# alibaba/unified-audio

Hardware: AMD Instinct MI355X
Metric: audio-seconds/sec H-Codec encode+decode @16kHz b=32 (higher is better)
Workload: dtype f32

## Files before the change

unified_audio_amd/csrc/conv_gemm.hip:

```cpp
#include <algorithm>
#include <cstdlib>
#include <type_traits>

#include "common.h"
#include "split_planes.h"

#ifndef QA_LOAD_AT
#define QA_LOAD_AT 0
#endif

#ifdef QA_TIMING
__device__ unsigned long long g_qa_timing[10];
extern "C" int qa_debug_timing(unsigned long long* out, int reset) {
    if (out && hipMemcpyFromSymbol(out, HIP_SYMBOL(g_qa_timing), sizeof(g_qa_timing)) != hipSuccess) return -1;
    if (reset) {
        unsigned long long z[10] = {0};
        if (hipMemcpyToSymbol(HIP_SYMBOL(g_qa_timing), z, sizeof(z)) != hipSuccess) return -1;
    }
    return 0;
}
#endif

namespace qa {

// ... 12 lines not shown
        f(std::integral_constant<int, I>{});
        static_for<N, I + 1>(f);
    }
}

constexpr int TAP_WIN = 8;

__device__ __forceinline__ float snake_f(float x, float a) {
    const float s = sinf(a * x);
    return x + s * s / (a + 1e-9f);
}
__device__ __forceinline__ f32x4 snake4(f32x4 v, const float* alpha, int n) {
    const f32x4 a = *reinterpret_cast<const f32x4*>(alpha + n);
    const f32x4 r = {snake_f(v.x, a.x), snake_f(v.y, a.y), snake_f(v.z, a.z), snake_f(v.w, a.w)};
    return r;
}

__device__ __forceinline__ f32x4 epilogue4(f32x4 v, const ConvParams& p, long long m, int n, f32x4 bias, f32x4 gamma) {
    v += bias;
    if (p.gate) {
        const f32x4 g = *reinterpret_cast<const f32x4*>(p.gate + m * p.ldg + n);
        v.x *= silu_f(g.x); v.y *= silu_f(g.y); v.z *= silu_f(g.z); v.w *= silu_f(g.w);
    }
    if (p.act == ACT_SNAKE) {
        v = snake4(v, p.alpha, n);
    } else if (p.act != ACT_NONE) {
        v.x = apply_act(v.x, p.act); v.y = apply_act(v.y, p.act); v.z = apply_act(v.z, p.act); v.w = apply_act(v.w, p.act);
    }
    if (p.gamma) v *= gamma;
    if (p.res) v += *reinterpret_cast<const f32x4*>(p.res + m * p.ldr + n);
    if (p.post_act == ACT_SNAKE) {
        v = snake4(v, p.alpha, n);
    } else if (p.post_act != ACT_NONE) {
        v.x = apply_act(v.x, p.post_act); v.y = apply_act(v.y, p.post_act); v.z = apply_act(v.z, p.post_act);
        v.w = apply_act(v.w, p.post_act);
    }
    if (p.y2) *reinterpret_cast<f32x4*>(p.y2 + m * p.ldy2 + n) = snake4(v, p.alpha2, n);
    if (p.rope && n < p.rope_n) {
        const int t = p.rope_pos0 + (int)(m % p.rope_T), i = (n % p.rope_hd) >> 1;
        const f32x4 cs = *reinterpret_cast<const f32x4*>(p.rope + ((long long)t * (p.rope_hd >> 1) + i) * 2);
        const f32x4 r = {v.x * cs.x - v.y * cs.y, v.y * cs.x + v.x * cs.y, v.z * cs.z - v.w * cs.w, v.w * cs.z + v.z * cs.w};
        v = r;
    }
    return v;
}

template <int BM, int BN, int WM, int WN, bool PRO_ELU, int BK = 32, bool LINEAR = false, int NPL = 0, bool PRE = false>
__global__ __launch_bounds__(256, conv_gemm_min_wg(BM, BN, BK, NPL > 0)) void conv_gemm_kernel(const ConvParams p_in) {
    constexpr bool SPLIT = NPL > 0;
    constexpr int NP = SPLIT ? NPL : 3;
    static_assert(NPL >= 0 && NPL <= 3, "0 = fp32 chain, else the number of bf16 planes");
    static_assert(SPLIT || !PRE, "a pre-split weight image feeds the bf16-plane instances only");
    ConvParams p = p_in;
    constexpr int LDS = BK + 4;
    constexpr int RPP = 256 / (BK / 4);
    constexpr int WTM = BM / WM, WTN = BN / WN;
    constexpr int TM = WTM / 32, TN = WTN / 32;
    constexpr int A_IT = BM / RPP, B_IT = BN / RPP;
    static_assert(WM * WN == 4, "4 waves per workgroup");
    static_assert(TM >= 1 && TN >= 1, "wave tile must hold at least one 32x32 MFMA tile");

    constexpr int SMEM_FLOATS = SPLIT ? 2 * (BM + BN) * 3 * BK / 2 : 2 * (BM + BN) * LDS;
    __shared__ __attribute__((aligned(16))) float smem[SMEM_FLOATS];
    __shared__ int s_tap[BM * TAP_WIN];
    float* sA = smem;
    float* sB = smem + 2 * BM * LDS;
    constexpr int PLANE_A = BM * BK * 2, PLANE_B = BN * BK * 2;
    constexpr int BUF_BYTES = 3 * (PLANE_A + PLANE_B);
    char* const sbytes = reinterpret_cast<char*>(smem);
    auto swz = [](int row, int slot) { return BK == 16 ? slot ^ ((row >> 3) & 1) : slot ^ ((row >> 2) & 3); };

    const int tid = threadIdx.x, lane = tid & 63, wave = tid >> 6;
    const int wm = wave / WN, wn = wave % WN;
    const int tiles_n = (p.N + BN - 1) / BN;
    int tile = blockIdx.x;
    if (p.xcd_swizzle) {
        const int nwg = gridDim.x, q = nwg >> 3, r = nwg & 7;
        const int xcd = tile & 7, local = tile >> 3;
        tile = (xcd < r ? xcd * (q + 1) : r * (q + 1) + (xcd - r) * q) + local;
    }
    int tm_i = tile / tiles_n, tn_i = tile % tiles_n;
    if (p.panel > 0 && tiles_n > p.panel) {
        const int tiles_m = (p.M + BM - 1) / BM;
        const int per_panel = tiles_m * p.panel;
        const int panel = tile / per_panel, r = tile - panel * per_panel;
        const int pw = min(p.panel, tiles_n - panel * p.panel);
        tm_i = r / pw;
        tn_i = panel * p.panel + (r - tm_i * pw);
    }
    const int m0 = tm_i * BM;
    const int n0 = tn_i * BN;

    const int ld_row = tid / (BK / 4);
    const int ld_c4 = (tid % (BK / 4)) * 4;

    const bool reflect = p.pad_mode == PAD_REFLECT;
    const int ldx_i = (int)p.ldx;
    const int t_virtual = p.T_in * (p.in_rep > 1 ? p.in_rep : 1);
    const int dil = p.dilation > 1 ? p.dilation : 1;
    auto build_taps = [&](int jbase) {
        for (int e = tid; e < BM * TAP_WIN; e += 256) {
            const int row = e / TAP_WIN, j = jbase + (e % TAP_WIN);
            const int m = min(m0 + row, p.M - 1);
            const int t = m % p.T_out;
            int len = t_virtual, lp = p.Lp;
            if (p.lens) {
                len = min(p.lens[m / p.T_out] * p.len_mul, t_virtual);
                lp = len <= p.max_pad ? p.max_pad + 1 : len;
            }
            int r = t * p.stride - p.pad_left + j * dil;
            const int rr = r < 0 ? -r : (r >= lp ? 2 * (lp - 1) - r : r);
            r = reflect ? rr : r;
            const bool ok = r >= 0 && r < len && j < p.ksize;
            const unsigned ru = ok ? (unsigned)r : 0u;
            const unsigned src = __umulhi(ru, p.rep_magic) + ru * p.rep_one;
            s_tap[e] = ok ? (int)(src * (unsigned)ldx_i) : -1;
        }
    };
    if (!LINEAR) build_taps(0);
    int jbase = 0;

    const float* a_ptr[A_IT];
    int a_tab[A_IT];
#pragma unroll
    for (int i = 0; i < A_IT; ++i) {
        const int m = min(m0 + ld_row + RPP * i, p.M - 1);
        a_ptr[i] = LINEAR ? p.x + (long long)m * p.ldx + ld_c4 : p.x + (long long)(m / p.T_out) * p.T_in * p.ldx + ld_c4;
        a_tab[i] = (ld_row + RPP * i) * TAP_WIN;
    }
    const float* b_ptr[B_IT];
    if constexpr (!PRE) {
#pragma unroll
        for (int i = 0; i < B_IT; ++i) {
            const int n = min(n0 + ld_row + RPP * i, p.N - 1);
            b_ptr[i] = p.w + (long long)n * p.K + ld_c4;
        }
    }
    constexpr int BP_BLOCK = 16 * NP;
    constexpr int BP_UNITS = BN * BK / 128 * BP_BLOCK, BP_IT = PRE ? BP_UNITS / 256 : 1;
    static_assert(!PRE || (BN == 128 && BP_UNITS % 256 == 0), "the image path exists for the 128-column tiles: every thread moves BP_IT whole units");
    const char* bp_ptr[BP_IT];
    int bp_lds[BP_IT];
    if constexpr (PRE) {
#pragma unroll
        for (int i = 0; i < BP_IT; ++i) {
            const int u = tid + 256 * i, v = u % BP_BLOCK;
            const int pl = v >> 4, slot = v % (BK / 8);
            const int row = u / BP_BLOCK * (128 / BK) + (v & 15) / (BK / 8);
            const int n = min(n0 + row, p.N - 1);
            bp_ptr[i] = static_cast<const char*>(p.wp) + plane_byte_offset((long long)n * p.K + slot * 8, pl);
            bp_lds[i] = 3 * PLANE_A + pl * PLANE_B + row * BK * 2 + swz(row, slot) * 16;
        }
    }
    const int nk = p.K / BK;

    f32x16 acc[TM][TN];
#pragma unroll
    for (int i = 0; i < TM; ++i)
#pragma unroll
        for (int j = 0; j < TN; ++j)
#pragma unroll
            for (int r = 0; r < 16; ++r) acc[i][j][r] = 0.f;

    f32x4 a_reg[A_IT], b_reg[B_IT];
    u32x4 bp_reg[BP_IT];
    float a_keep[A_IT];

#define QA_LOAD_GLOBAL(KC)                                                                                     \
    {                                                                                                          \
        const int k0_ = (KC) * BK;                                                                             \
        if (LINEAR) {                                                                                          \
            _Pragma("unroll") for (int i = 0; i < A_IT; ++i) a_reg[i] = *reinterpret_cast<const f32x4*>(a_ptr[i] + k0_); \
        } else {                                                                                               \
            const int j_ = k0_ / p.C_in;                                                                       \
            const int c_ = k0_ - j_ * p.C_in;                                                                  \
            if (j_ >= jbase + TAP_WIN) {                          \
                jbase = j_;                                                                                    \
                build_taps(jbase);                                                                             \
                __syncthreads();                                                                               \
            }                                                                                                  \
            _Pragma("unroll") for (int i = 0; i < A_IT; ++i) {                                                 \
                const int off_ = s_tap[a_tab[i] + (j_ - jbase)];                                               \
                a_keep[i] = off_ >= 0 ? 1.f : 0.f;                                                             \
                a_reg[i] = *reinterpret_cast<const f32x4*>(a_ptr[i] + (unsigned)(max(off_, 0) + c_));          \
            }                                                                                                  \
        }                                                                                                      \
        if constexpr (PRE) {                                                                                   \
            _Pragma("unroll") for (int i = 0; i < BP_IT; ++i)                                                  \
                bp_reg[i] = *reinterpret_cast<const u32x4*>(bp_ptr[i] + (long long)(KC) * (BK * 6)); \
        } else {                                                                                               \
            _Pragma("unroll") for (int i = 0; i < B_IT; ++i) b_reg[i] = *reinterpret_cast<const f32x4*>(b_ptr[i] + k0_); \
        }                                                                                                      \
    }
#define QA_STORE_LDS(BUF)                                                                                      \
    { if constexpr (SPLIT) {                                                                                   \
        char* a_ = sbytes + (BUF) * BUF_BYTES;                                                                 \
        const int sl_ = ld_c4 >> 3, in_ = (ld_c4 & 7) * 2;                                                     \
        _Pragma("unroll") for (int i = 0; i < A_IT; ++i) {                                                     \
            f32x4 v = LINEAR ? a_reg[i] : a_reg[i] * a_keep[i];                                                \
            if (PRO_ELU) {                                                                                     \
                v.x = elu_f(v.x); v.y = elu_f(v.y); v.z = elu_f(v.z); v.w = elu_f(v.w);                        \
            }                                                                                                  \
            u32x2 h_, m_, l_;                                                                                  \
            split4_planes<NP>(v, h_, m_, l_);                                                                  \
            const int r_ = ld_row + RPP * i, o_ = r_ * BK * 2 + swz(r_, sl_) * 16 + in_;                       \
            *reinterpret_cast<u32x2*>(a_ + o_) = h_;                                                           \
            if constexpr (NP >= 2) *reinterpret_cast<u32x2*>(a_ + PLANE_A + o_) = m_;                          \
            if constexpr (NP == 3) *reinterpret_cast<u32x2*>(a_ + 2 * PLANE_A + o_) = l_;                      \
        }                                                                                                      \
        if constexpr (PRE) {                                                                                   \
            _Pragma("unroll") for (int i = 0; i < BP_IT; ++i)                                                  \
                *reinterpret_cast<u32x4*>(a_ + bp_lds[i]) = bp_reg[i];                                         \
        } else {                                                                                               \
        char* b_ = a_ + 3 * PLANE_A;                                                                           \
        _Pragma("unroll") for (int i = 0; i < B_IT; ++i) {                                                     \
            u32x2 h_, m_, l_;                                                                                  \
            split4_planes<NP>(b_reg[i], h_, m_, l_);                                                           \
            const int r_ = ld_row + RPP * i, o_ = r_ * BK * 2 + swz(r_, sl_) * 16 + in_;                       \
            *reinterpret_cast<u32x2*>(b_ + o_) = h_;                                                           \
            if constexpr (NP >= 2) *reinterpret_cast<u32x2*>(b_ + PLANE_B + o_) = m_;                          \
            if constexpr (NP == 3) *reinterpret_cast<u32x2*>(b_ + 2 * PLANE_B + o_) = l_;                      \
        } }                                                                                                    \
    } else {                                                                                                   \
        float* a_ = sA + (BUF) * BM * LDS;                                                                     \
        float* b_ = sB + (BUF) * BN * LDS;                                                                     \
        _Pragma("unroll") for (int i = 0; i < A_IT; ++i) {                                                     \
            f32x4 v = LINEAR ? a_reg[i] : a_reg[i] * a_keep[i];                                                \
            if (PRO_ELU) {                                                                                     \
                v.x = elu_f(v.x); v.y = elu_f(v.y); v.z = elu_f(v.z); v.w = elu_f(v.w);                        \
            }                                                                                                  \
            *reinterpret_cast<f32x4*>(a_ + (ld_row + RPP * i) * LDS + ld_c4) = v;                              \
        }                                                                                                      \
        _Pragma("unroll") for (int i = 0; i < B_IT; ++i)                                                       \
            *reinterpret_cast<f32x4*>(b_ + (ld_row + RPP * i) * LDS + ld_c4) = b_reg[i];                       \
    } }

    __syncthreads();
    QA_LOAD_GLOBAL(0)
    QA_STORE_LDS(0)
    __syncthreads();

    const int frag_row = lane & 31;
    const int frag_k = (lane >> 5) * 4;
#ifdef QA_TIMING
    const long long tbegin = __builtin_readcyclecounter();
    const unsigned long long rbegin = __builtin_amdgcn_s_memrealtime();
#endif
    constexpr int NKK = BK / 8;
    if constexpr (SPLIT) {
        constexpr int NG = BK / 16;
        const int sl_h = lane >> 5;
        int a_off[TM], b_off[TN];
#pragma unroll
        for (int i = 0; i < TM; ++i) {
            const int r = wm * WTM + i * 32 + frag_row;
            a_off[i] = r * BK * 2 + swz(r, sl_h) * 16;
        }
#pragma unroll
        for (int j = 0; j < TN; ++j) {
            const int r = wn * WTN + j * 32 + frag_row;
            b_off[j] = 3 * PLANE_A + r * BK * 2 + swz(r, sl_h) * 16;
        }
        for (int kc = 0; kc < nk; ++kc) {
            const int cur = kc & 1;
            const int nxt = min(kc + 1, nk - 1);
            const char* base = sbytes + cur * BUF_BYTES;
#pragma unroll
            for (int g = 0; g < NG; ++g) {
                bf16x8 af[NP][TM], bf[NP][TN];
#pragma unroll
                for (int pl = 0; pl < NP; ++pl) {
#pragma unroll
                    for (int i = 0; i < TM; ++i)
                        af[pl][i] = *reinterpret_cast<const bf16x8*>(base + pl * PLANE_A + (a_off[i] ^ (32 * g)));
#pragma unroll
                    for (int j = 0; j < TN; ++j)
                        bf[pl][j] = *reinterpret_cast<const bf16x8*>(base + pl * PLANE_B + (b_off[j] ^ (32 * g)));
                }
                if (g == 0) QA_LOAD_GLOBAL(nxt)
                if (g == NG - 1) QA_STORE_LDS(cur ^ 1)
                if constexpr (NP == 3) {
#pragma unroll
                for (int q = 0; q < 6; ++q)
#pragma unroll
                    for (int i = 0; i < TM; ++i)
#pragma unroll
                        for (int j = 0; j < TN; ++j)
                            acc[i][j] = __builtin_amdgcn_mfma_f32_32x32x16_bf16(bf[PAIR_B[q]][j], af[PAIR_A[q]][i], acc[i][j], 0, 0, 0);
                } else {
                    static_for<6>([&](auto q_c) {
                        constexpr int q = decltype(q_c)::value;
                        if constexpr (pair_kept(q, NP)) {
#pragma unroll
                            for (int i = 0; i < TM; ++i)
#pragma unroll
                                for (int j = 0; j < TN; ++j)
                                    acc[i][j] = __builtin_amdgcn_mfma_f32_32x32x16_bf16(bf[PAIR_B[q]][j], af[PAIR_A[q]][i], acc[i][j], 0, 0, 0);
                        }
                    });
                }
                __builtin_amdgcn_sched_barrier(0);
            }
            __syncthreads();
        }
    } else
    for (int kc = 0; kc < nk; ++kc) {
        const int cur = kc & 1;
        const int nxt = min(kc + 1, nk - 1);
        const float* a = sA + cur * BM * LDS + (wm * WTM + frag_row) * LDS + frag_k;
        const float* b = sB + cur * BN * LDS + (wn * WTN + frag_row) * LDS + frag_k;
        f32x4 af[2][TM], bf[2][TN];
#pragma unroll
        for (int i = 0; i < TM; ++i) af[0][i] = *reinterpret_cast<const f32x4*>(a + i * 32 * LDS);
#pragma unroll
        for (int j = 0; j < TN; ++j) bf[0][j] = *reinterpret_cast<const f32x4*>(b + j * 32 * LDS);
#pragma unroll
        for (int kk = 0; kk < NKK; ++kk) {
            const int cb = kk & 1, nb = cb ^ 1;
            if (kk < NKK - 1) {
#pragma unroll
                for (int i = 0; i < TM; ++i) af[nb][i] = *reinterpret_cast<const f32x4*>(a + i * 32 * LDS + (kk + 1) * 8);
#pragma unroll
                for (int j = 0; j < TN; ++j) bf[nb][j] = *reinterpret_cast<const f32x4*>(b + j * 32 * LDS + (kk + 1) * 8);
            }
            if (kk == QA_LOAD_AT) QA_LOAD_GLOBAL(nxt)
            if (kk == NKK - 1) QA_STORE_LDS(cur ^ 1)
#pragma unroll
            for (int i = 0; i < TM; ++i)
#pragma unroll
                for (int j = 0; j < TN; ++j) {
                    acc[i][j] = __builtin_amdgcn_mfma_f32_32x32x2f32(bf[cb][j].x, af[cb][i].x, acc[i][j], 0, 0, 0);
                    acc[i][j] = __builtin_amdgcn_mfma_f32_32x32x2f32(bf[cb][j].y, af[cb][i].y, acc[i][j], 0, 0, 0);
                    acc[i][j] = __builtin_amdgcn_mfma_f32_32x32x2f32(bf[cb][j].z, af[cb][i].z, acc[i][j], 0, 0, 0);
                    acc[i][j] = __builtin_amdgcn_mfma_f32_32x32x2f32(bf[cb][j].w, af[cb][i].w, acc[i][j], 0, 0, 0);
                }
            __builtin_amdgcn_sched_barrier(0);
        }
        __syncthreads();
    }
#ifdef QA_TIMING
    const long long tloop = __builtin_readcyclecounter();
#endif
#undef QA_LOAD_GLOBAL
#undef QA_STORE_LDS

    constexpr int EP_LD = BN + 4;
    constexpr int EP_ROWS = WM * 32;
    constexpr int EP_C4 = BN / 4;
    static_assert(EP_ROWS * EP_LD <= 2 * (BM + BN) * LDS, "epilogue staging must fit in the operand buffers");
    static_assert(256 % EP_C4 == 0, "a thread keeps its column group across iterations");
    static_assert(EP_C4 % 8 == 0, "arg-min epilogue: the 8 lanes of a 32-column group are consecutive lanes of one wave");
    float* stage = smem;
    const int row_l = lane & 31, col_h = 4 * (lane >> 5);
    const int ep_c4 = tid % EP_C4, ep_r0 = tid / EP_C4;
    const int ep_n = n0 + 4 * ep_c4;
    const f32x4 zero4 = {0.f, 0.f, 0.f, 0.f}, one4 = {1.f, 1.f, 1.f, 1.f};
    f32x4 bias4 = zero4, gamma4 = one4;
    if (p.vec_epi && ep_n < p.N) {
        if (p.bias) bias4 = *reinterpret_cast<const f32x4*>(p.bias + ep_n);
        if (p.gamma) gamma4 = *reinterpret_cast<const f32x4*>(p.gamma + ep_n);
    }
    static_for<TM>([&](auto i_c) {
        constexpr int i = decltype(i_c)::value;
        __syncthreads();
#pragma unroll
        for (int j = 0; j < TN; ++j)
#pragma unroll
            for (int g = 0; g < 4; ++g) {
                const f32x4 v = {acc[i][j][4 * g], acc[i][j][4 * g + 1], acc[i][j][4 * g + 2], acc[i][j][4 * g + 3]};
                *reinterpret_cast<f32x4*>(stage + (wm * 32 + row_l) * EP_LD + wn * WTN + j * 32 + 8 * g + col_h) = v;
            }
        __syncthreads();
#pragma unroll 1
        for (int r = ep_r0; r < EP_ROWS; r += 256 / EP_C4) {
            const long long m = m0 + (r >> 5) * WTM + i * 32 + (r & 31);
            if (p.am_dist) {
                float best = INFINITY;
                int bi = 0x7fffffff;
                if (m < p.M && ep_n < p.N) {
                    const f32x4 sv = *reinterpret_cast<const f32x4*>(stage + r * EP_LD + 4 * ep_c4);
                    const f32x4 e4 = *reinterpret_cast<const f32x4*>(p.am_e2 + ep_n);
                    const float xx = p.am_x2[m];
#pragma unroll
                    for (int e = 0; e < 4; ++e) {
                        const float dist = (xx - 2.f * sv[e]) + e4[e];
                        if (dist < best) {
                            best = dist;
                            bi = ep_n + e;
                        }
                    }
                }
#pragma unroll
                for (int o = 1; o < 8; o <<= 1) {
                    const float d2 = __shfl_xor(best, o, 64);
                    const int i2 = __shfl_xor(bi, o, 64);
                    if (d2 < best || (d2 == best && i2 < bi)) {
                        best = d2;
                        bi = i2;
                    }
                }
                if ((ep_c4 & 7) == 0 && m < p.M && ep_n < p.N) {
                    p.am_dist[m * p.am_ld + (ep_n >> 5)] = best;
                    p.am_idx[m * p.am_ld + (ep_n >> 5)] = bi;
                }
                continue;
            }
            if (m >= p.M || ep_n >= p.N) continue;
            f32x4 v = *reinterpret_cast<const f32x4*>(stage + r * EP_LD + 4 * ep_c4);
            if (p.vec_epi) {
                v = epilogue4(v, p, m, ep_n, bias4, gamma4);
                *reinterpret_cast<f32x4*>(p.y + m * p.ldy + ep_n) = v;
            } else {
                for (int e = 0; e < 4 && ep_n + e < p.N; ++e) {
                    const int n = ep_n + e;
                    float u = v[e] + (p.bias ? p.bias[n] : 0.f);
                    if (p.gate) u = silu_f(p.gate[m * p.ldg + n]) * u;
                    u = apply_act(u, p.act);
                    if (p.gamma) u *= p.gamma[n];
                    if (p.res) u += p.res[m * p.ldr + n];
                    u = apply_act(u, p.post_act);
                    p.y[m * p.ldy + n] = u;
                }
            }
        }
// ... 1 lines not shown
#ifdef QA_TIMING
    if (lane == 0) {
        const long long tend = __builtin_readcyclecounter();
        atomicAdd(&g_qa_timing[4], (unsigned long long)(tend - tloop));
        atomicAdd(&g_qa_timing[5], (unsigned long long)(tend - tbegin));
        atomicAdd(&g_qa_timing[6], 1ULL);
        atomicAdd(&g_qa_timing[7], (unsigned long long)nk);
        atomicAdd(&g_qa_timing[8], __builtin_amdgcn_s_memrealtime() - rbegin);
    }
#endif
}

static bool is_linear(const ConvParams& p) {
    return knob(K_GEMM_LINEAR) != 0 && p.ksize == 1 && p.stride == 1 && p.pad_left == 0 && p.in_rep <= 1 && p.T_in == p.T_out && p.dilation <= 1;
}

constexpr int prof_cfg(int bm, int bn) {
    return bm == 256 ? PROF_CFG_256x128 : bm == 64 ? (bn == 64 ? PROF_CFG_64x64 : PROF_CFG_64x128) : bn == 32 ? PROF_CFG_128x32 : bn == 64 ? PROF_CFG_128x64 : PROF_CFG_128x128;
}

static int gemm_planes(const ConvParams& p) {
    const long long math = knob(K_GEMM_MATH);
    return math == 0 || p.math_fp32 ? 0 : math == 2 ? 2 : math == 3 ? 1 : 3;
}

template <int BM, int BN, int WM, int WN, bool ELU, int BK, bool LIN>
static void launch_instance(const ConvParams& p, long long tiles, hipStream_t stream) {
    constexpr bool IMAGE = BN == 128;
    const bool image = IMAGE && p.wp;
    void (*kernel)(const ConvParams) = nullptr;
    switch (gemm_planes(p)) {
        case 0: kernel = conv_gemm_kernel<BM, BN, WM, WN, ELU, BK, LIN, 0, false>; break;
        case 1: kernel = image ? conv_gemm_kernel<BM, BN, WM, WN, ELU, BK, LIN, 1, IMAGE> : conv_gemm_kernel<BM, BN, WM, WN, ELU, BK, LIN, 1, false>; break;
        case 2: kernel = image ? conv_gemm_kernel<BM, BN, WM, WN, ELU, BK, LIN, 2, IMAGE> : conv_gemm_kernel<BM, BN, WM, WN, ELU, BK, LIN, 2, false>; break;
        default: kernel = image ? conv_gemm_kernel<BM, BN, WM, WN, ELU, BK, LIN, 3, IMAGE> : conv_gemm_kernel<BM, BN, WM, WN, ELU, BK, LIN, 3, false>; break;
    }
    hipLaunchKernelGGL(kernel, dim3((unsigned)tiles), dim3(256), 0, stream, p);
}

static thread_local int t_gemm_lanes = 1;
GemmLanes::GemmLanes(int n) : prev(t_gemm_lanes) { t_gemm_lanes = n > 1 ? n : 1; }
GemmLanes::~GemmLanes() { t_gemm_lanes = prev; }
static bool takes_bk16(int bm, int bn, long long tiles, int K, int C_in, bool elu) {
    return bm == 256 ||
           (bn >= 64 && !elu && ((K <= knob(K_GEMM_BK16) && tiles * t_gemm_lanes >= knob(K_GEMM_BK16_MIN_TILES)) || C_in % 32 != 0));
}

template <int BM, int BN, int WM, int WN>
static int launch_cfg(const ConvParams& p, hipStream_t stream) {
    QA_REQUIRE(p.prologue == ACT_NONE || p.prologue == ACT_ELU, "conv_gemm: prologue %d unsupported", p.prologue);
    const long long tiles = ceil_div(p.M, BM) * ceil_div(p.N, BN);
    const bool linear = is_linear(p), elu = p.prologue == ACT_ELU;
    const bool bk16 = takes_bk16(BM, BN, tiles, p.K, p.C_in, elu);
    const int bk = bk16 ? 16 : 32;
    const bool table = BM != 256 && (!linear || elu);
    QA_REQUIRE(p.K % bk == 0 && (!table || p.C_in % bk == 0),
               "conv_gemm: the %dx%d tile's BK = %d K chunk does not divide K=%d / C_in=%d", BM, BN, bk, p.K, p.C_in);
    const bool prof = profile_enabled();
    if (prof) {
        const double n = p.algo_n ? p.algo_n : p.N, k = p.algo_k ? p.algo_k : p.K;
        const double out_elems = p.am_dist ? 2.0 * (double)p.M * p.am_ld + p.M + n
                                            : (double)p.M * n * (1.0 + (p.res ? 1.0 : 0.0) + (p.gate ? 1.0 : 0.0));
        const double elems = (double)p.B * p.T_in * p.C_in + n * k + out_elems;
        profile_record_begin(prof_cfg(BM, BN), 2.0 * (double)p.M * n * k, 4.0 * elems, stream, &p);
    }
    if constexpr (BM == 256) QA_REQUIRE(linear && !elu, "conv_gemm: the 256 x 128 tile exists for LINEAR layers only");
    constexpr int BK16 = BN >= 64 ? 16 : 32;
    if (bk16 && linear) launch_instance<BM, BN, WM, WN, false, BK16, true>(p, tiles, stream);
    else if constexpr (BM != 256) {
        if (bk16) launch_instance<BM, BN, WM, WN, false, BK16, false>(p, tiles, stream);
        else if (elu) launch_instance<BM, BN, WM, WN, true, 32, false>(p, tiles, stream);
        else if (linear) launch_instance<BM, BN, WM, WN, false, 32, true>(p, tiles, stream);
        else launch_instance<BM, BN, WM, WN, false, 32, false>(p, tiles, stream);
    }
    if (prof) profile_record_end(stream);
    QA_LAUNCH_CHECK();
    return QA_OK;
}

struct TileQuery {
    long long M, N, K;
    int C_in;
    bool lin, elu, split;
    bool image;
    int share;
};
static int workgroups_per_cu(int cfg, bool bk16, bool split) {
    switch (cfg) {
        case PROF_CFG_128x128: return bk16 ? 3 : split ? 1 : 2;
        case PROF_CFG_64x128: return bk16 ? 4 : 2;
        case PROF_CFG_128x64: return bk16 ? 4 : 2;
        case PROF_CFG_64x64: return bk16 ? 5 : split ? 3 : 4;
        case PROF_CFG_256x128: return 2;
        default: return split ? 2 : 3;
    }
}
static double tile_cost(const TileQuery& t, int cfg, int bm, int bn, double eff) {
    constexpr double kTile = 128.0 * 128.0, kRamp = 0.22, kLaunch = 0.27 * 512.0;
    const long long tiles = ceil_div(t.M, bm) * ceil_div(t.N, bn);
    const long long w = workgroups_per_cu(cfg, takes_bk16(bm, bn, tiles, (int)t.K, t.C_in, t.elu), t.split);
    const long long n = tiles * (t.share > 1 ? t.share : 1), cap = 256 * w;
    const long long rounds = ceil_div(n, cap), m = n - (rounds - 1) * cap;
    double last = 0.5 * ((double)ceil_div(m, 256) + (double)m / 256.0);
    if (last < 1.0) last = 1.0;
    return kTile * kLaunch + (double)t.K * ((double)bm * bn / eff * ((double)(w * (rounds - 1)) + last) + kRamp * kTile * (double)rounds);
}
static double tile_cost_r4(const TileQuery& t, int bm, int bn, double eff) {
    const long long tiles = ceil_div(t.M, bm) * ceil_div(t.N, bn);
    return (double)ceil_div(tiles, 256) * bm * bn / eff * (tiles <= 256 ? 1.25 : 1.0);
}
static int choose_tile(const TileQuery& t) {
    int cfg = (int)knob(K_GEMM_CFG);
    if (cfg < 0) {
        if (t.N <= 32) cfg = PROF_CFG_128x32;
        else if (t.N <= 64) cfg = PROF_CFG_128x64;
        else {
            struct Cand { int cfg, bm, bn; double eff6, eff32; };
            static const Cand cands[] = {{PROF_CFG_128x128, 128, 128, 1.0, 1.0}, {PROF_CFG_64x128, 64, 128, 0.85, 0.914},
                                         {PROF_CFG_128x64, 128, 64, 0.80, 0.913}, {PROF_CFG_64x64, 64, 64, 0.69, 0.871}};
            double best = 0.0;
            cfg = PROF_CFG_128x128;
            const long long eff256 = knob(K_GEMM_256);
            const bool r4 = t.split && !t.image;
            if (eff256 > 0 && t.lin && t.M >= 8000 && t.N >= 1024) {
                best = r4 ? tile_cost_r4(t, 256, 128, eff256 / 1000.0) : tile_cost(t, PROF_CFG_256x128, 256, 128, eff256 / 1000.0);
                cfg = PROF_CFG_256x128;
            }
            for (const Cand& c : cands) {
                const double cost = r4 ? tile_cost_r4(t, c.bm, c.bn, c.eff32) : tile_cost(t, c.cfg, c.bm, c.bn, t.split ? c.eff6 : c.eff32);
                if (best == 0.0 || cost < best * 0.995) {
                    best = cost;
                    cfg = c.cfg;
                }
            }
        }
    }
    if (cfg == PROF_CFG_128x32 && t.C_in % 32 != 0) return PROF_CFG_128x64;
    if ((cfg == PROF_CFG_256x128 && !t.lin) || cfg >= PROF_NCFG) return PROF_CFG_128x128;
    return cfg;
}
static int choose_tile(const ConvParams& p) {
    const bool elu = p.prologue == ACT_ELU;
    return choose_tile(TileQuery{p.M, p.N, p.K, p.C_in, is_linear(p) && !elu, elu, knob(K_GEMM_MATH) != 0 && !p.math_fp32, p.wp != nullptr, 1});
}

int launch_conv_gemm(const ConvParams& p, hipStream_t stream) {
    QA_REQUIRE(p.K % 16 == 0 && p.C_in % 16 == 0, "conv_gemm: K=%d / C_in=%d must be multiples of 16", p.K, p.C_in);
    QA_REQUIRE(p.C_in % 32 == 0 || (p.N > 32 && p.prologue != ACT_ELU),
               "conv_gemm: C_in=%d is not a multiple of 32 (only supported for N > 32 without the ELU prologue)", p.C_in);
    QA_REQUIRE((p.ldx % 4) == 0, "conv_gemm: ldx=%lld must be a multiple of 4 floats", p.ldx);
    QA_REQUIRE((long long)p.T_in * p.ldx < (1LL << 31), "conv_gemm: one batch item spans %lld floats (limit 2^31)",
               (long long)p.T_in * p.ldx);
    QA_REQUIRE(((uintptr_t)p.x % 16) == 0 && ((uintptr_t)p.w % 16) == 0, "conv_gemm: x / w must be 16-byte aligned");
    if (p.M <= 0 || p.N <= 0) return QA_OK;
    QA_REQUIRE(ceil_div(p.M, 64) * ceil_div(p.N, 32) < (1LL << 31), "conv_gemm: grid too large");
    auto al16 = [](const void* ptr) { return ((uintptr_t)ptr % 16) == 0; };
    const bool vec_epi = p.N % 4 == 0 && p.ldy % 4 == 0 && al16(p.y) && (!p.bias || al16(p.bias)) && (!p.gamma || al16(p.gamma)) &&
                         (!p.res || (p.ldr % 4 == 0 && al16(p.res))) && (!p.gate || (p.ldg % 4 == 0 && al16(p.gate)));
    QA_REQUIRE(p.in_rep <= 1 || p.pad_mode == PAD_ZERO, "conv_gemm: in_rep needs zero padding");
    const bool snake = p.act == ACT_SNAKE || p.post_act == ACT_SNAKE;
    QA_REQUIRE((!snake && !p.y2) || (vec_epi && (!snake || (p.alpha && al16(p.alpha))) &&
                                     (!p.y2 || (p.alpha2 && al16(p.alpha2) && al16(p.y2) && p.ldy2 % 4 == 0))),
               "conv_gemm: Snake activation / second output need the float4 epilogue and 16-byte aligned alpha vectors");
    QA_REQUIRE(p.dilation <= 1 || (p.pad_mode == PAD_ZERO && p.in_rep <= 1), "conv_gemm: dilation needs zero padding");
    QA_REQUIRE(!p.lens || (p.len_mul >= 1 && p.max_pad >= 0), "conv_gemm: per-clip lengths need len_mul >= 1");
    QA_REQUIRE(!p.am_dist || (vec_epi && p.am_idx && p.am_x2 && p.am_e2 && al16(p.am_e2) && p.am_ld >= (p.N + 31) / 32 && !p.y2),
               "conv_gemm: the arg-min epilogue needs N %% 4 == 0, x2 / e2 / dist / idx and am_ld >= ceil(N / 32)");
    QA_REQUIRE(!p.rope || (vec_epi && p.rope_hd % 4 == 0 && p.rope_n % 4 == 0 && p.rope_T > 0 && al16(p.rope)),
               "conv_gemm: fused RoPE needs the float4 epilogue (N, strides, pointers multiples of 4 / 16 B)");
    ConvParams q = p;
    q.xcd_swizzle = (int)knob(K_GEMM_XCD);
    q.panel = (int)knob(K_GEMM_PANEL);
    q.wp = knob(K_GEMM_PRESPLIT) != 0 ? weight_planes_find(p.w, (long long)p.N * p.K) : nullptr;
    q.vec_epi = vec_epi;
    q.rep_one = p.in_rep > 1 ? 0u : 1u;
    q.rep_magic = p.in_rep > 1 ? (unsigned)(((1ULL << 32) + p.in_rep - 1) / p.in_rep) : 0u;

    switch (choose_tile(q)) {
        case PROF_CFG_128x32: return launch_cfg<128, 32, 4, 1>(q, stream);
        case PROF_CFG_128x64: return launch_cfg<128, 64, 2, 2>(q, stream);
        case PROF_CFG_64x128: return launch_cfg<64, 128, 1, 4>(q, stream);
        case PROF_CFG_64x64: return launch_cfg<64, 64, 2, 2>(q, stream);
        case PROF_CFG_256x128: return launch_cfg<256, 128, 2, 2>(q, stream);
        default: return launch_cfg<128, 128, 2, 2>(q, stream);
    }
}

int conv_params_from_args(const qa_conv_args& a, ConvParams* out) {
    ConvParams p{};
    QA_REQUIRE(a.x && a.w && a.y, "conv1d_cl: x, w, y must be non-null");
    QA_REQUIRE(a.B > 0 && a.T_in > 0 && a.C_in > 0 && a.N > 0 && a.T_out >= 0, "conv1d_cl: bad shape");
    QA_REQUIRE(a.ksize >= 1 && a.stride >= 1 && a.pad_left >= 0 && a.pad_right >= 0, "conv1d_cl: bad geometry");
    QA_REQUIRE(a.B * a.T_out < (1LL << 31) && a.ksize * a.C_in < (1LL << 31), "conv1d_cl: shape too large");
    p.x = a.x; p.w = a.w; p.bias = a.bias; p.gamma = a.gamma; p.res = a.residual; p.gate = a.gate; p.y = a.y;
    p.ldx = a.ldx ? a.ldx : a.C_in;
    p.ldy = a.ldy ? a.ldy : a.N;
    p.ldr = a.ldr ? a.ldr : a.N;
    p.ldg = a.ldg ? a.ldg : a.N;
    p.B = (int)a.B; p.T_in = (int)a.T_in; p.C_in = (int)a.C_in; p.T_out = (int)a.T_out; p.N = (int)a.N;
    p.K = (int)(a.ksize * a.C_in);
    p.M = (int)(a.B * a.T_out);
    p.ksize = a.ksize; p.stride = a.stride; p.pad_left = a.pad_left; p.pad_mode = a.pad_mode;
// ... 22 lines not shown
```

unified_audio_amd/csrc/knobs.h:

```cpp
#pragma once
#include <cstdint>

namespace qa {

#define QA_KNOB_TABLE(X)                                                                                                           \
    X(SERIAL, "QA_SERIAL", 0, "1: no internal stream concurrency (every kernel alone on the device; = qa_set_serial)")           \
    X(GEMM_CFG, "QA_GEMM_CFG", -1, "force the conv_gemm tile: 0 = 128x32, 1 = 128x64, 2 = 128x128, 3 = 64x128, 4 = 64x64, 5 = 256x128 (LINEAR layers; else 128x128) (-1: cost model)")             \
    X(GEMM_256, "QA_GEMM_256", 0, "r06 experiment: 256x128 block tile (4 waves, 4x2 accumulators each) for LINEAR layers with M >= 8000 and N >= 1024; value = its efficiency relative to 128x128 in 1/1000 for the cost model (0: never chosen; QA_GEMM_CFG=5 forces it)") \
    X(GEMM_BK16, "QA_GEMM_BK16", 1 << 30, "largest K that takes the BK = 16 K-chunk variant")                                     \
    X(GEMM_BK16_MIN_TILES, "QA_GEMM_BK16_MIN_TILES", 384, "fewest tiles of a launch that take BK = 16")                          \
    X(GEMM_MATH, "QA_GEMM_MATH", 1, "conv_gemm arithmetic: 1 = split-6 (operands split into three bf16 planes, six v_mfma_f32_32x32x16_bf16 per 16-wide k group, fp32 accumulation), 0 = the fp32 chain (v_mfma_f32_32x32x2_f32); opt-in reduced precision: 2 = split-3 (two planes, products hm, mh, hh: operands exact to 2^-16), 3 = bf16 (one plane, one product: bf16 operands, fp32 accumulation); any other value = split-6; launches marked math_fp32 (the UniSE LM) keep the fp32 chain") \
    X(GEMM_PRESPLIT, "QA_GEMM_PRESPLIT", 1, "split-6 weights from a pre-split image: a weight store builds the three bf16 planes of all its weights once, at load (6 bytes per weight beside the fp32 blob; not built when 0 at load time), and conv_gemm's 128-column tiles copy them into LDS instead of splitting the weight tile in the K loop (narrower tiles keep the in-loop split); 0 at launch = ignore the image and split in the loop; same bits either way") \
    X(GEMM_LINEAR, "QA_GEMM_LINEAR", 1, "table-free K loop for ksize-1 layers")                                                  \
    X(GEMM_XCD, "QA_GEMM_XCD", 1, "XCD-aware tile order")                                                                        \
    X(GEMM_PANEL, "QA_GEMM_PANEL", 8, "conv_gemm tile order: column panels of this many tiles, row tiles fastest inside a panel (0: column tiles fastest over the whole row; 8: +4 % on N >= 4096 shapes, +1.2 % on H-Codec 2.0)") \
    X(ATT_MATH, "QA_ATT_MATH", 1, "attention arithmetic: 1 = split-6 (Q, K, V and the probabilities as three bf16 planes, six v_mfma_f32_32x32x16_bf16 per 16-wide k group, fp32 accumulation), 0 = the fp32 chain (v_mfma_f32_32x32x2_f32); the UniSE LM keeps the fp32 chain either way") \
    X(ATT_DEBUG, "QA_ATT_DEBUG", 0, "attention_kernel debug bits, both forms: 1 always rescale, 2 extra barrier per tile, 4 wait for the prefetch at once, 8 no wave-uniform tile skip, 16 mask every tile; the split-6 form (SPLIT) only (tests): 32 / 64 / 128 zero the h / m / l plane of the operands selected by 256 Q, 512 K, 1024 V, 2048 P (none of the four: all)") \
    X(AGG_LAST_ROWS, "QA_AGG_LAST_ROWS", 1, "H-Codec 1.5 encode: the last layer of each aggregator stack runs attention, out_proj, LayerNorm 2, lin1 and lin2 on the G query rows per clip only (the rows the read-out keeps); 0 = the full last layer; same bits either way") \
    X(BATCH_SPLIT, "QA_BATCH_SPLIT", 1, "H-Codec: a one-stream phase as two half-batch lanes on two streams - clips [0, ceil(B / 2)) on the caller's stream, the rest on an internal one, enqueued layer by layer and joined before the next recurrence (bit mask): 1 = the H-Codec 1.5 bottleneck transformer (32 x 10 s: 97.5 -> 96.1 ms per step); 0 = one lane; one lane as well for B = 1, under QA_SERIAL and with taps on; same bits either way") \
    X(BATCH_SPLIT_MIN_ROWS, "QA_BATCH_SPLIT_MIN_ROWS", 500, "QA_BATCH_SPLIT: fewest rows (clips x frames) of the smaller lane at which a region is split (10 s clips: lanes of 250 rows lose 0.5 ms, 500 rows gain 0.3 ms; tests: 0)") \
    X(SEANET_FUSED, "QA_SEANET_FUSED", 1, "fused conv0 + first SEANet residual block")                                           \
    X(MIMI_ROPE_WINDOW, "QA_MIMI_ROPE_WINDOW", 8192, "mimi streaming: positions covered by the RoPE table before the rolling window takes over (tests shrink it)") \
    X(LSTM_GRAPH, "QA_LSTM_GRAPH", 1, "replay the T step launches of an LSTM call from a cached hipGraph")                       \
    X(LSTM_PERSISTENT, "QA_LSTM_PERSISTENT", -1, "persistent recurrence kernel: -1 auto (d >= 1536), 0 off, 1 on for every supported width") \
    X(LSTM_XCD, "QA_LSTM_XCD", 1, "XCD-local LSTM recurrence for d = 512 / 768 (lstm_team_kernel with one team per XCD: one launch, W_hh in the registers of every XCD's 32 CUs, sequences dealt to the XCDs, 32-member step barrier per XCD): 0 off (the per-step kernels), 1 agent-scope hand-off forms, 2 XCD-local forms (h stores that stay in the XCD's L2; H-Codec 1.0: 42.7 against 43.3 ms)") \
    X(LSTM_TEAM, "QA_LSTM_TEAM", 1, "team recurrence for d = 1024 (lstm_team_kernel, one launch: 4 teams of 64 workgroups, W_hh resident in registers, 8 sequences per team, agent-scope hand-offs; H-Codec 1.5 decoder: 134.1 -> 128.3 ms per step, profiles/r04_lstm_team_ab.txt): 0 = the per-step kernels") \
    X(LSTM_SPIN_LIMIT, "QA_LSTM_SPIN_LIMIT", 1 << 21, "persistent recurrence: polls of a barrier word before the barrier is declared broken") \
    X(LSTM_FAULT, "QA_LSTM_FAULT", 0, "1 (tests): the step barrier of every in-launch recurrence (lstm_persistent_kernel, lstm_team_kernel) waits for one workgroup more than exists, like a starved launch") \
    X(LM_GRAPH, "QA_LM_GRAPH", 0, "1: replay one captured decode step per token")                                                \
    X(LM_MLP_FUSED, "QA_LM_MLP_FUSED", 1, "decode step: gate/up + SwiGLU + down of 16 activation columns per workgroup in one launch emitting K-slice partials, summed by a reduce launch (0: separate gate/up and down launches)") \
    X(LM_PF, "QA_LM_PF", 7, "decode step: cross-launch L2 weight prefetch planes (bit mask; lm_decode.h PfArgs): 1 qkv launch -> o_proj weights, 2 o_proj launch -> fused-MLP weights, 4 MLP launch -> next layer's qkv weights (last layer: the head slice), 8 head launch -> layer 0 qkv weights") \
    X(LM_ROWSPLIT, "QA_LM_ROWSPLIT", 3, "decode step at 9 .. 16 sequences: two 8-row groups instead of one 16-row group in the qkv launch (bit 1) and the fused-MLP launch (bit 2)") \
    X(LM_CHAINS, "QA_LM_CHAINS", 0, "generate: number of concurrent chains on internal streams (0: ceil(B / 64) - one chain serves up to 64 sequences, two row groups of 32 per launch; a count that would put more than 64 sequences into a chain is raised)") \
    X(LM_SCORE_ROWS, "QA_LM_SCORE_ROWS", 4096, "qa_lm_score: target rows per output_head launch (the logits buffer holds this many rows of the full vocabulary; any value gives the same bits)")

enum Knob {
#define QA_KNOB_ENUM(id, name, def, doc) K_##id,
    QA_KNOB_TABLE(QA_KNOB_ENUM)
#undef QA_KNOB_ENUM
        K_COUNT
};

long long knob(Knob k);
void knob_set(Knob k, long long v);

}
```

Baseline: 3329.

## Switch split-bf16 conv GEMM to 16x16x32 MFMA with 32-wide K chunks

The split-plane (bf16x3) path of conv_gemm now uses v_mfma_f32_16x16x32_bf16 on 16x16 accumulator tiles instead of 32x32x16. It loads 32-wide K chunks, handles a 16-wide K tail by zeroing the upper half, and adds a single-LDS-buffer variant for the former BK=16 selection. The aim is to halve the K-loop trip count, give the MFMA more K per instruction and cut LDS traffic per FLOP, at the cost of more accumulator registers and added tail and addressing logic. The epilogue and launch checks are adapted so C_in values that are multiples of 16 are accepted on the split path.

Result: faster. 3497, median of 6 (+5.1%).

```diff
diff --git a/unified_audio_amd/csrc/conv_gemm.hip b/unified_audio_amd/csrc/conv_gemm.hip
--- a/unified_audio_amd/csrc/conv_gemm.hip
+++ b/unified_audio_amd/csrc/conv_gemm.hip
@@ -88,23 +88,25 @@
     static_assert(NPL >= 0 && NPL <= 3, "0 = fp32 chain, else the number of bf16 planes");
     static_assert(SPLIT || !PRE, "a pre-split weight image feeds the bf16-plane instances only");
     ConvParams p = p_in;
+    constexpr int CK = SPLIT ? 32 : BK;
+    constexpr bool ONE_BUF = SPLIT && BK == 16;
     constexpr int LDS = BK + 4;
-    constexpr int RPP = 256 / (BK / 4);
+    constexpr int RPP = 256 / (CK / 4);
     constexpr int WTM = BM / WM, WTN = BN / WN;
     constexpr int TM = WTM / 32, TN = WTN / 32;
     constexpr int A_IT = BM / RPP, B_IT = BN / RPP;
     static_assert(WM * WN == 4, "4 waves per workgroup");
     static_assert(TM >= 1 && TN >= 1, "wave tile must hold at least one 32x32 MFMA tile");
 
-    constexpr int SMEM_FLOATS = SPLIT ? 2 * (BM + BN) * 3 * BK / 2 : 2 * (BM + BN) * LDS;
+    constexpr int SMEM_FLOATS = SPLIT ? (ONE_BUF ? 1 : 2) * (BM + BN) * 3 * CK / 2 : 2 * (BM + BN) * LDS;
     __shared__ __attribute__((aligned(16))) float smem[SMEM_FLOATS];
     __shared__ int s_tap[BM * TAP_WIN];
     float* sA = smem;
     float* sB = smem + 2 * BM * LDS;
-    constexpr int PLANE_A = BM * BK * 2, PLANE_B = BN * BK * 2;
+    constexpr int PLANE_A = BM * CK * 2, PLANE_B = BN * CK * 2;
     constexpr int BUF_BYTES = 3 * (PLANE_A + PLANE_B);
     char* const sbytes = reinterpret_cast<char*>(smem);
-    auto swz = [](int row, int slot) { return BK == 16 ? slot ^ ((row >> 3) & 1) : slot ^ ((row >> 2) & 3); };
+    auto swz = [](int row, int slot) { return slot ^ ((0 - (row >> 2)) & 3); };
 
     const int tid = threadIdx.x, lane = tid & 63, wave = tid >> 6;
     const int wm = wave / WN, wn = wave % WN;
@@ -127,8 +129,10 @@
     const int m0 = tm_i * BM;
     const int n0 = tn_i * BN;
 
-    const int ld_row = tid / (BK / 4);
-    const int ld_c4 = (tid % (BK / 4)) * 4;
+    const int ld_row = tid / (CK / 4);
+    const int ld_c4 = (tid % (CK / 4)) * 4;
+    const bool ld_hi = SPLIT && ld_c4 >= 16, bp_hi = (tid & 2) != 0;
+    const bool k_tail = SPLIT && (p.K & 16) != 0;
 
     const bool reflect = p.pad_mode == PAD_REFLECT;
     const int ldx_i = (int)p.ldx;
@@ -173,7 +177,7 @@
         }
     }
     constexpr int BP_BLOCK = 16 * NP;
-    constexpr int BP_UNITS = BN * BK / 128 * BP_BLOCK, BP_IT = PRE ? BP_UNITS / 256 : 1;
+    constexpr int BP_UNITS = BN * CK / 128 * BP_BLOCK, BP_IT = PRE ? BP_UNITS / 256 : 1;
     static_assert(!PRE || (BN == 128 && BP_UNITS % 256 == 0), "the image path exists for the 128-column tiles: every thread moves BP_IT whole units");
     const char* bp_ptr[BP_IT];
     int bp_lds[BP_IT];
@@ -181,14 +185,14 @@
 #pragma unroll
         for (int i = 0; i < BP_IT; ++i) {
             const int u = tid + 256 * i, v = u % BP_BLOCK;
-            const int pl = v >> 4, slot = v % (BK / 8);
-            const int row = u / BP_BLOCK * (128 / BK) + (v & 15) / (BK / 8);
+            const int pl = v >> 4, slot = v % (CK / 8);
+            const int row = u / BP_BLOCK * (128 / CK) + (v & 15) / (CK / 8);
             const int n = min(n0 + row, p.N - 1);
             bp_ptr[i] = static_cast<const char*>(p.wp) + plane_byte_offset((long long)n * p.K + slot * 8, pl);
-            bp_lds[i] = 3 * PLANE_A + pl * PLANE_B + row * BK * 2 + swz(row, slot) * 16;
-        }
-    }
-    const int nk = p.K / BK;
+            bp_lds[i] = 3 * PLANE_A + pl * PLANE_B + row * CK * 2 + swz(row, slot) * 16;
+        }
+    }
+    const int nk = (p.K + CK - 1) / CK;
 
     f32x16 acc[TM][TN];
 #pragma unroll
@@ -197,6 +201,14 @@
         for (int j = 0; j < TN; ++j)
 #pragma unroll
             for (int r = 0; r < 16; ++r) acc[i][j][r] = 0.f;
+    constexpr int TM16 = WTM / 16, TN16 = WTN / 16;
+    f32x4 acc4[SPLIT ? TM16 : 1][SPLIT ? TN16 : 1];
+    if constexpr (SPLIT) {
+#pragma unroll
+        for (int i = 0; i < TM16; ++i)
+#pragma unroll
+            for (int j = 0; j < TN16; ++j) acc4[i][j] = f32x4{0.f, 0.f, 0.f, 0.f};
+    }
 
     f32x4 a_reg[A_IT], b_reg[B_IT];
     u32x4 bp_reg[BP_IT];
@@ -204,34 +216,54 @@
 
 #define QA_LOAD_GLOBAL(KC)                                                                                     \
     {                                                                                                          \
-        const int k0_ = (KC) * BK;                                                                             \
+        const int k0_ = (KC) * CK;                                                                             \
+        const bool tl_ = k_tail && (KC) == nk - 1;             \
+        const int kt_ = k0_ - (tl_ && ld_hi ? 16 : 0);          \
         if (LINEAR) {                                                                                          \
-            _Pragma("unroll") for (int i = 0; i < A_IT; ++i) a_reg[i] = *reinterpret_cast<const f32x4*>(a_ptr[i] + k0_); \
+            _Pragma("unroll") for (int i = 0; i < A_IT; ++i) a_reg[i] = *reinterpret_cast<const f32x4*>(a_ptr[i] + kt_); \
         } else {                                                                                               \
-            const int j_ = k0_ / p.C_in;                                                                       \
-            const int c_ = k0_ - j_ * p.C_in;                                                                  \
-            if (j_ >= jbase + TAP_WIN) {                          \
-                jbase = j_;                                                                                    \
+            const int j0_ = k0_ / p.C_in;                                                                      \
+            const int c0_ = k0_ - j0_ * p.C_in;                                                                \
+            int j1_ = j0_, c1_ = c0_;                                                                          \
+            if (SPLIT && (p.C_in & 16)) {        \
+                const int kh_ = tl_ ? k0_ : k0_ + 16;                                                          \
+                j1_ = kh_ / p.C_in;                                                                            \
+                c1_ = kh_ - j1_ * p.C_in - 16;                                                                 \
+            }                                                                                                  \
+            if (j1_ >= jbase + TAP_WIN) {                         \
+                jbase = j0_;                                                                                   \
                 build_taps(jbase);                                                                             \
                 __syncthreads();                                                                               \
             }                                                                                                  \
+            const int j_ = ld_hi ? j1_ : j0_, c_ = ld_hi ? c1_ : c0_;                                          \
             _Pragma("unroll") for (int i = 0; i < A_IT; ++i) {                                                 \
                 const int off_ = s_tap[a_tab[i] + (j_ - jbase)];                                               \
                 a_keep[i] = off_ >= 0 ? 1.f : 0.f;                                                             \
-                a_reg[i] = *reinterpret_cast<const f32x4*>(a_ptr[i] + (unsigned)(max(off_, 0) + c_));          \
+                a_reg[i] = *reinterpret_cast<const f32x4*>(a_ptr[i] + (max(off_, 0) + c_));                    \
             }                                                                                                  \
         }                                                                                                      \
         if constexpr (PRE) {                                                                                   \
+            const long long bo_ = (long long)(KC) * (CK * 6) - (tl_ && bp_hi ? 2 * PLANE_GROUP_BYTES : 0);     \
             _Pragma("unroll") for (int i = 0; i < BP_IT; ++i)                                                  \
-                bp_reg[i] = *reinterpret_cast<const u32x4*>(bp_ptr[i] + (long long)(KC) * (BK * 6)); \
+                bp_reg[i] = *reinterpret_cast<const u32x4*>(bp_ptr[i] + bo_);                                  \
         } else {                                                                                               \
-            _Pragma("unroll") for (int i = 0; i < B_IT; ++i) b_reg[i] = *reinterpret_cast<const f32x4*>(b_ptr[i] + k0_); \
+            _Pragma("unroll") for (int i = 0; i < B_IT; ++i) b_reg[i] = *reinterpret_cast<const f32x4*>(b_ptr[i] + kt_); \
         }                                                                                                      \
     }
-#define QA_STORE_LDS(BUF)                                                                                      \
+#define QA_STORE_LDS(BUF, KC)                                                                                  \
     { if constexpr (SPLIT) {                                                                                   \
         char* a_ = sbytes + (BUF) * BUF_BYTES;                                                                 \
         const int sl_ = ld_c4 >> 3, in_ = (ld_c4 & 7) * 2;                                                     \
+        if (k_tail && (KC) == nk - 1) {        \
+            const f32x4 z4_ = {0.f, 0.f, 0.f, 0.f};                                                            \
+            const u32x4 zu_ = {0u, 0u, 0u, 0u};                                                                \
+            _Pragma("unroll") for (int i = 0; i < A_IT; ++i) a_reg[i] = ld_hi ? z4_ : a_reg[i];                \
+            if constexpr (PRE) {                                                                               \
+                _Pragma("unroll") for (int i = 0; i < BP_IT; ++i) bp_reg[i] = bp_hi ? zu_ : bp_reg[i];         \
+            } else {                                                                                           \
+                _Pragma("unroll") for (int i = 0; i < B_IT; ++i) b_reg[i] = ld_hi ? z4_ : b_reg[i];            \
+            }                                                                                                  \
+        }                                                                                                      \
         _Pragma("unroll") for (int i = 0; i < A_IT; ++i) {                                                     \
             f32x4 v = LINEAR ? a_reg[i] : a_reg[i] * a_keep[i];                                                \
             if (PRO_ELU) {                                                                                     \
@@ -239,7 +271,7 @@
             }                                                                                                  \
             u32x2 h_, m_, l_;                                                                                  \
             split4_planes<NP>(v, h_, m_, l_);                                                                  \
-            const int r_ = ld_row + RPP * i, o_ = r_ * BK * 2 + swz(r_, sl_) * 16 + in_;                       \
+            const int r_ = ld_row + RPP * i, o_ = r_ * CK * 2 + swz(r_, sl_) * 16 + in_;                       \
             *reinterpret_cast<u32x2*>(a_ + o_) = h_;                                                           \
             if constexpr (NP >= 2) *reinterpret_cast<u32x2*>(a_ + PLANE_A + o_) = m_;                          \
             if constexpr (NP == 3) *reinterpret_cast<u32x2*>(a_ + 2 * PLANE_A + o_) = l_;                      \
@@ -252,7 +284,7 @@
         _Pragma("unroll") for (int i = 0; i < B_IT; ++i) {                                                     \
             u32x2 h_, m_, l_;                                                                                  \
             split4_planes<NP>(b_reg[i], h_, m_, l_);                                                           \
-            const int r_ = ld_row + RPP * i, o_ = r_ * BK * 2 + swz(r_, sl_) * 16 + in_;                       \
+            const int r_ = ld_row + RPP * i, o_ = r_ * CK * 2 + swz(r_, sl_) * 16 + in_;                       \
             *reinterpret_cast<u32x2*>(b_ + o_) = h_;                                                           \
             if constexpr (NP >= 2) *reinterpret_cast<u32x2*>(b_ + PLANE_B + o_) = m_;                          \
             if constexpr (NP == 3) *reinterpret_cast<u32x2*>(b_ + 2 * PLANE_B + o_) = l_;                      \
@@ -273,7 +305,7 @@
 
     __syncthreads();
     QA_LOAD_GLOBAL(0)
-    QA_STORE_LDS(0)
+    QA_STORE_LDS(0, 0)
     __syncthreads();
 
     const int frag_row = lane & 31;
@@ -284,60 +316,58 @@
 #endif
     constexpr int NKK = BK / 8;
     if constexpr (SPLIT) {
-        constexpr int NG = BK / 16;
-        const int sl_h = lane >> 5;
-        int a_off[TM], b_off[TN];
-#pragma unroll
-        for (int i = 0; i < TM; ++i) {
-            const int r = wm * WTM + i * 32 + frag_row;
-            a_off[i] = r * BK * 2 + swz(r, sl_h) * 16;
-        }
-#pragma unroll
-        for (int j = 0; j < TN; ++j) {
-            const int r = wn * WTN + j * 32 + frag_row;
-            b_off[j] = 3 * PLANE_A + r * BK * 2 + swz(r, sl_h) * 16;
+        constexpr int RB = BM == 256 ? 4 : 1;
+        constexpr int STORE_J = TN16 > 1 ? 1 : 0;
+        const int fr = lane & 15, sl = lane >> 4;
+        int a_off[TM16], b_off[TN16];
+#pragma unroll
+        for (int i = 0; i < TM16; ++i) {
+            const int r = wm * WTM + i * 16 + fr;
+            a_off[i] = r * CK * 2 + swz(r, sl) * 16;
+        }
+#pragma unroll
+        for (int j = 0; j < TN16; ++j) {
+            const int r = wn * WTN + j * 16 + fr;
+            b_off[j] = 3 * PLANE_A + r * CK * 2 + swz(r, sl) * 16;
         }
         for (int kc = 0; kc < nk; ++kc) {
-            const int cur = kc & 1;
+            const int cur = ONE_BUF ? 0 : kc & 1;
             const int nxt = min(kc + 1, nk - 1);
             const char* base = sbytes + cur * BUF_BYTES;
-#pragma unroll
-            for (int g = 0; g < NG; ++g) {
-                bf16x8 af[NP][TM], bf[NP][TN];
-#pragma unroll
-                for (int pl = 0; pl < NP; ++pl) {
-#pragma unroll
-                    for (int i = 0; i < TM; ++i)
-                        af[pl][i] = *reinterpret_cast<const bf16x8*>(base + pl * PLANE_A + (a_off[i] ^ (32 * g)));
-#pragma unroll
-                    for (int j = 0; j < TN; ++j)
-                        bf[pl][j] = *reinterpret_cast<const bf16x8*>(base + pl * PLANE_B + (b_off[j] ^ (32 * g)));
-                }
-                if (g == 0) QA_LOAD_GLOBAL(nxt)
-                if (g == NG - 1) QA_STORE_LDS(cur ^ 1)
-                if constexpr (NP == 3) {
-#pragma unroll
-                for (int q = 0; q < 6; ++q)
-#pragma unroll
-                    for (int i = 0; i < TM; ++i)
-#pragma unroll
-                        for (int j = 0; j < TN; ++j)
-                            acc[i][j] = __builtin_amdgcn_mfma_f32_32x32x16_bf16(bf[PAIR_B[q]][j], af[PAIR_A[q]][i], acc[i][j], 0, 0, 0);
-                } else {
+            QA_LOAD_GLOBAL(nxt)
+            static_for<RB>([&](auto rb_c) {
+                constexpr int i0 = decltype(rb_c)::value * (TM16 / RB);
+                bf16x8 af[NP][TM16 / RB];
+#pragma unroll
+                for (int pl = 0; pl < NP; ++pl)
+#pragma unroll
+                    for (int i = 0; i < TM16 / RB; ++i) af[pl][i] = *reinterpret_cast<const bf16x8*>(base + pl * PLANE_A + a_off[i0 + i]);
+#pragma unroll
+                for (int j = 0; j < TN16; ++j) {
+                    bf16x8 bf[NP];
+#pragma unroll
+                    for (int pl = 0; pl < NP; ++pl) bf[pl] = *reinterpret_cast<const bf16x8*>(base + pl * PLANE_B + b_off[j]);
+                    if (!ONE_BUF && i0 + TM16 / RB == TM16 && j == STORE_J) QA_STORE_LDS(cur ^ 1, nxt)
                     static_for<6>([&](auto q_c) {
                         constexpr int q = decltype(q_c)::value;
                         if constexpr (pair_kept(q, NP)) {
 #pragma unroll
-                            for (int i = 0; i < TM; ++i)
-#pragma unroll
-                                for (int j = 0; j < TN; ++j)
-                                    acc[i][j] = __builtin_amdgcn_mfma_f32_32x32x16_bf16(bf[PAIR_B[q]][j], af[PAIR_A[q]][i], acc[i][j], 0, 0, 0);
+                            for (int i = 0; i < TM16 / RB; ++i)
+                                acc4[i0 + i][j] = __builtin_amdgcn_mfma_f32_16x16x32_bf16(bf[PAIR_B[q]], af[PAIR_A[q]][i], acc4[i0 + i][j], 0, 0, 0);
                         }
                     });
                 }
-                __builtin_amdgcn_sched_barrier(0);
+            });
+            __builtin_amdgcn_sched_barrier(0);
+            if constexpr (ONE_BUF) {
+                if (kc + 1 < nk) {
+                    __syncthreads();
+                    QA_STORE_LDS(0, nxt)
+                    __syncthreads();
+                }
+            } else {
+                __syncthreads();
             }
-            __syncthreads();
         }
     } else
     for (int kc = 0; kc < nk; ++kc) {
@@ -360,7 +390,7 @@
                 for (int j = 0; j < TN; ++j) bf[nb][j] = *reinterpret_cast<const f32x4*>(b + j * 32 * LDS + (kk + 1) * 8);
             }
             if (kk == QA_LOAD_AT) QA_LOAD_GLOBAL(nxt)
-            if (kk == NKK - 1) QA_STORE_LDS(cur ^ 1)
+            if (kk == NKK - 1) QA_STORE_LDS(cur ^ 1, nxt)
 #pragma unroll
             for (int i = 0; i < TM; ++i)
 #pragma unroll
@@ -399,6 +429,13 @@
     static_for<TM>([&](auto i_c) {
         constexpr int i = decltype(i_c)::value;
         __syncthreads();
+        if constexpr (SPLIT) {
+#pragma unroll
+            for (int h = 0; h < 2; ++h)
+#pragma unroll
+                for (int j = 0; j < TN16; ++j)
+                    *reinterpret_cast<f32x4*>(stage + (wm * 32 + h * 16 + (lane & 15)) * EP_LD + wn * WTN + j * 16 + 4 * (lane >> 4)) = acc4[2 * i + h][j];
+        } else {
 #pragma unroll
         for (int j = 0; j < TN; ++j)
 #pragma unroll
@@ -406,6 +443,7 @@
                 const f32x4 v = {acc[i][j][4 * g], acc[i][j][4 * g + 1], acc[i][j][4 * g + 2], acc[i][j][4 * g + 3]};
                 *reinterpret_cast<f32x4*>(stage + (wm * 32 + row_l) * EP_LD + wn * WTN + j * 32 + 8 * g + col_h) = v;
             }
+        }
         __syncthreads();
 #pragma unroll 1
         for (int r = ep_r0; r < EP_ROWS; r += 256 / EP_C4) {
@@ -513,10 +551,10 @@
     const long long tiles = ceil_div(p.M, BM) * ceil_div(p.N, BN);
     const bool linear = is_linear(p), elu = p.prologue == ACT_ELU;
     const bool bk16 = takes_bk16(BM, BN, tiles, p.K, p.C_in, elu);
-    const int bk = bk16 ? 16 : 32;
+    const int bk = bk16 || gemm_planes(p) > 0 ? 16 : 32;
     const bool table = BM != 256 && (!linear || elu);
     QA_REQUIRE(p.K % bk == 0 && (!table || p.C_in % bk == 0),
-               "conv_gemm: the %dx%d tile's BK = %d K chunk does not divide K=%d / C_in=%d", BM, BN, bk, p.K, p.C_in);
+               "conv_gemm: the %dx%d tile's K chunk needs K=%d / C_in=%d to be multiples of %d", BM, BN, p.K, p.C_in, bk);
     const bool prof = profile_enabled();
     if (prof) {
         const double n = p.algo_n ? p.algo_n : p.N, k = p.algo_k ? p.algo_k : p.K;
@@ -607,8 +645,8 @@
 
 int launch_conv_gemm(const ConvParams& p, hipStream_t stream) {
     QA_REQUIRE(p.K % 16 == 0 && p.C_in % 16 == 0, "conv_gemm: K=%d / C_in=%d must be multiples of 16", p.K, p.C_in);
-    QA_REQUIRE(p.C_in % 32 == 0 || (p.N > 32 && p.prologue != ACT_ELU),
-               "conv_gemm: C_in=%d is not a multiple of 32 (only supported for N > 32 without the ELU prologue)", p.C_in);
+    QA_REQUIRE(p.C_in % 32 == 0 || gemm_planes(p) > 0 || (p.N > 32 && p.prologue != ACT_ELU),
+               "conv_gemm: C_in=%d is not a multiple of 32 (the fp32 chain supports that only for N > 32 without the ELU prologue)", p.C_in);
     QA_REQUIRE((p.ldx % 4) == 0, "conv_gemm: ldx=%lld must be a multiple of 4 floats", p.ldx);
     QA_REQUIRE((long long)p.T_in * p.ldx < (1LL << 31), "conv_gemm: one batch item spans %lld floats (limit 2^31)",
                (long long)p.T_in * p.ldx);
diff --git a/unified_audio_amd/csrc/knobs.h b/unified_audio_amd/csrc/knobs.h
--- a/unified_audio_amd/csrc/knobs.h
+++ b/unified_audio_amd/csrc/knobs.h
@@ -7,9 +7,9 @@
     X(SERIAL, "QA_SERIAL", 0, "1: no internal stream concurrency (every kernel alone on the device; = qa_set_serial)")           \
     X(GEMM_CFG, "QA_GEMM_CFG", -1, "force the conv_gemm tile: 0 = 128x32, 1 = 128x64, 2 = 128x128, 3 = 64x128, 4 = 64x64, 5 = 256x128 (LINEAR layers; else 128x128) (-1: cost model)")             \
     X(GEMM_256, "QA_GEMM_256", 0, "r06 experiment: 256x128 block tile (4 waves, 4x2 accumulators each) for LINEAR layers with M >= 8000 and N >= 1024; value = its efficiency relative to 128x128 in 1/1000 for the cost model (0: never chosen; QA_GEMM_CFG=5 forces it)") \
-    X(GEMM_BK16, "QA_GEMM_BK16", 1 << 30, "largest K that takes the BK = 16 K-chunk variant")                                     \
+    X(GEMM_BK16, "QA_GEMM_BK16", 1 << 30, "largest K that takes the BK = 16 K-chunk variant (fp32 chain: 16-wide chunks; split forms: one LDS buffer of 32 k instead of two)")                                     \
     X(GEMM_BK16_MIN_TILES, "QA_GEMM_BK16_MIN_TILES", 384, "fewest tiles of a launch that take BK = 16")                          \
-    X(GEMM_MATH, "QA_GEMM_MATH", 1, "conv_gemm arithmetic: 1 = split-6 (operands split into three bf16 planes, six v_mfma_f32_32x32x16_bf16 per 16-wide k group, fp32 accumulation), 0 = the fp32 chain (v_mfma_f32_32x32x2_f32); opt-in reduced precision: 2 = split-3 (two planes, products hm, mh, hh: operands exact to 2^-16), 3 = bf16 (one plane, one product: bf16 operands, fp32 accumulation); any other value = split-6; launches marked math_fp32 (the UniSE LM) keep the fp32 chain") \
+    X(GEMM_MATH, "QA_GEMM_MATH", 1, "conv_gemm arithmetic: 1 = split-6 (operands split into three bf16 planes, six v_mfma_f32_16x16x32_bf16 per 32-wide k group, fp32 accumulation), 0 = the fp32 chain (v_mfma_f32_32x32x2_f32); opt-in reduced precision: 2 = split-3 (two planes, products hm, mh, hh: operands exact to 2^-16), 3 = bf16 (one plane, one product: bf16 operands, fp32 accumulation); any other value = split-6; launches marked math_fp32 (the UniSE LM) keep the fp32 chain") \
     X(GEMM_PRESPLIT, "QA_GEMM_PRESPLIT", 1, "split-6 weights from a pre-split image: a weight store builds the three bf16 planes of all its weights once, at load (6 bytes per weight beside the fp32 blob; not built when 0 at load time), and conv_gemm's 128-column tiles copy them into LDS instead of splitting the weight tile in the K loop (narrower tiles keep the in-loop split); 0 at launch = ignore the image and split in the loop; same bits either way") \
     X(GEMM_LINEAR, "QA_GEMM_LINEAR", 1, "table-free K loop for ksize-1 layers")                                                  \
     X(GEMM_XCD, "QA_GEMM_XCD", 1, "XCD-aware tile order")                                                                        \
```
